# Jamy-L/Handheld-Multi-Frame-Super-Resolution

Measured on AMD Instinct MI355X. Metric: output Mpix/s for 12MP x 20-frame x2 SR burst; max-abs diff vs reference, higher is better.
Workload: dtype f32

## Files before the change

### handheld-multi-frame-super-resolution_amd/csrc/hhsr_kernels.hip

```cpp
#include "hhsr_common.h"


struct CovParams {
    double alpha, beta, k_detail, k_denoise, D_th, D_tr, k_stretch, k_shrink;
    int law;
    double r_D_tr, inv_k_shrink;
};

__device__ __forceinline__ double div_by(double a, double b, double r) {
    const double q = a * r;
    return fma(fma(-b, q, a), r, q);
}

#ifndef HHSR_FAST_SQRT
#define HHSR_FAST_SQRT 1
#endif
__device__ __forceinline__ double sqrt_pos(double t) {
#if HHSR_FAST_SQRT
    const double y = __builtin_amdgcn_rsq(t);
    double g = t * y, h = 0.5 * y;
    const double r = fma(-h, g, 0.5);
    g = fma(g, r, g);
    h = fma(h, r, h);
    const double d = fma(-g, g, t);
    return fma(d, h, g);
#else
    return sqrt(t);
#endif
}

#ifndef HHSR_FAST_DIV
#define HHSR_FAST_DIV 1
#endif
__device__ __forceinline__ float div_f32(float x, float y) {
#if HHSR_FAST_DIV
    const float r = __builtin_amdgcn_rcpf(y), q = x * r;
    return fmaf(fmaf(-y, q, x), r, q);
#else
    return x / y;
#endif
}

__device__ __forceinline__ float gat1(float v, double alpha, double c0, double two_over_alpha) {
    const double t = fmax(alpha * (double)v + c0, 1.0e-300);
    return (float)(two_over_alpha * sqrt_pos(t));
}

template <int SGP>
__device__ __forceinline__ float4 quad_cov(const float* __restrict__ sg, int ly, int lx, int qy, int qx, int gh, int gw,
                                           const CovParams& P) {
    float T00 = 0.f, T01 = 0.f, T11 = 0.f;
#pragma unroll
    for (int i = 0; i < 2; ++i) {
#pragma unroll
        for (int j = 0; j < 2; ++j) {
            const int gy_ = qy - 1 + i, gx_ = qx - 1 + j;
            if (gy_ >= 0 && gy_ < gh - 1 && gx_ >= 0 && gx_ < gw - 1) {
                const float g00 = sg[(ly + i) * SGP + lx + j], g01 = sg[(ly + i) * SGP + lx + j + 1];
                const float g10 = sg[(ly + i + 1) * SGP + lx + j], g11 = sg[(ly + i + 1) * SGP + lx + j + 1];
                const float t0a = -0.5f * g00 + 0.5f * g01, t0b = -0.5f * g10 + 0.5f * g11;
                const float t1a = 0.5f * g00 + 0.5f * g01, t1b = 0.5f * g10 + 0.5f * g11;
                const float vx = 0.5f * t0a + 0.5f * t0b;
                const float vy = -0.5f * t1a + 0.5f * t1b;
                T00 += vx * vx;
                T01 += vx * vy;
                T11 += vy * vy;
            }
        }
    }
    const float b = -(T00 + T11);
    const float c = T00 * T11 - T01 * T01;
    const float bb = b * b;
    double delta = (double)bb - 4.0 * (double)c;
    delta = delta > 0.0 ? delta : 0.0;
    const double sq = delta > 0.0 ? sqrt_pos(delta) : 0.0;
    const double r1 = (-(double)b + sq) / 2.0, r2 = (-(double)b - sq) / 2.0;
    float l1, l2;
    if (fabs(r1) >= fabs(r2)) {
        l1 = (float)r1;
        l2 = (float)r2;
    } else {
        l1 = (float)r2;
        l2 = (float)r1;
    }
    float e1x, e1y, e2x, e2y;
    if (T01 == 0.f && T00 == T11) {
        e1x = 1.f; e1y = 0.f; e2x = 0.f; e2y = 1.f;
    } else {
        const float a0 = T00 + T01 - l2, a1 = T01 + T11 - l2;
        if (a0 == 0.f) {
            e1x = a0; e1y = 1.f; e2x = 1.f; e2y = 0.f;
        } else if (a1 == 0.f) {
            e1x = 1.f; e1y = a1; e2x = 0.f; e2y = 1.f;
        } else {
            const float nrm = sqrtf(a0 * a0 + a1 * a1);
            e1x = div_f32(a0, nrm);
            e1y = div_f32(a1, nrm);
            const float sgn = copysignf(1.f, e1x);
            e2y = fabsf(e1x);
            e2x = -e1y * sgn;
        }
    }
    const double A = 1.0 + (double)sqrtf(div_f32(l1 - l2, l1 + l2));
    double D = 1.0 - div_by((double)sqrtf(l1), P.D_tr, P.r_D_tr) + P.D_th;
    D = D > 0.0 ? D : 0.0;
    D = D < 1.0 ? D : 1.0;
    double k1d, k2d;
    if (P.law == 0) {
        if (A > 1.95) {
            k1d = P.inv_k_shrink;
            k2d = P.k_stretch;
        } else {
            k1d = 1.0;
            k2d = 1.0;
        }
    } else {
        k1d = 1.0 + A / 2.0 * (P.inv_k_shrink - 1.0);
        k2d = 1.0 + A / 2.0 * (P.k_stretch - 1.0);
    }
    const float k1 = (float)(P.k_detail * ((1.0 - D) * k1d + D * P.k_denoise));
    const float k2 = (float)(P.k_detail * ((1.0 - D) * k2d + D * P.k_denoise));
    const float k1s = k1 * k1, k2s = k2 * k2;
    float4 o;
    o.x = k1s * e1x * e1x + k2s * e2x * e2x;
    o.y = k1s * e1x * e1y + k2s * e2x * e2y;
    o.z = o.y;
    o.w = k1s * e1y * e1y + k2s * e2y * e2y;
    return o;
}

constexpr int FS_TX = 32, FS_TY = 16, FS_P = FS_TX + 2 + 1, FS_N = (FS_TY + 2) * (FS_TX + 2);
constexpr int FS_IT = (FS_N + 255) / 256;

struct FsCfa {
    uint8_t c[4];
};
struct FsFrames {
    const float* raw[HHSR_MAX_BATCH];
    float* means[HHSR_MAX_BATCH];
    float* vars[HHSR_MAX_BATCH];
    float4* covs[HHSR_MAX_BATCH];
};

struct FrameStatsArgs {
    const float* raw;
    int pitch, gh, gw;
    FsCfa cfa;
    double rwb[3];
    double rwbk[4];
    int pat;
    int unit_wb;
    float* means;
    float* vars;
    float4* covs;
    CovParams P;
};

template <bool STATS, bool COV>
__global__ void __launch_bounds__(256) k_frame_stats(FrameStatsArgs A, FsFrames fr) {
    A.raw = fr.raw[blockIdx.z];
    A.means = fr.means[blockIdx.z];
    A.vars = fr.vars[blockIdx.z];
    A.covs = fr.covs[blockIdx.z];
    __shared__ float s_ch[STATS ? 3 : 1][STATS ? FS_TY + 2 : 1][FS_P];
    __shared__ float s_g[COV ? (FS_TY + 2) * FS_P : 1];
    const int bid = xcd_remap(blockIdx.y * gridDim.x + blockIdx.x, gridDim.x * gridDim.y);
    const int qx0 = (bid % gridDim.x) * FS_TX, qy0 = (bid / gridDim.x) * FS_TY;
    const int gh = A.gh, gw = A.gw;
    const double c0 = 3.0 / 8.0 * A.P.alpha * A.P.alpha + A.P.beta;
    const double toa = 2.0 / A.P.alpha;
    float2 va[FS_IT], vb[FS_IT];
#pragma unroll
    for (int u = 0; u < FS_IT; ++u) {
        const int p = min(threadIdx.x + 256 * u, FS_N - 1);
        const int i = p / (FS_TX + 2), j = p - i * (FS_TX + 2);
        const int qy = clampi(qy0 + i - 1, 0, gh - 1), qx = clampi(qx0 + j - 1, 0, gw - 1);
        va[u] = *reinterpret_cast<const float2*>(A.raw + (size_t)(2 * qy) * A.pitch + 2 * qx);
        vb[u] = *reinterpret_cast<const float2*>(A.raw + (size_t)(2 * qy + 1) * A.pitch + 2 * qx);
    }
#pragma unroll
    for (int u = 0; u < FS_IT; ++u) {
        const int p = threadIdx.x + 256 * u;
        if (p < FS_N) {
            const int i = p / (FS_TX + 2), j = p - i * (FS_TX + 2);
            const float v[4] = {va[u].x, va[u].y, vb[u].x, vb[u].y};
            if (STATS) {
                float ch[3] = {0.f, 0.f, 0.f};
                const double x0 = (double)v[0] * A.rwbk[0], x1 = (double)v[1] * A.rwbk[1];
                const double x2 = (double)v[2] * A.rwbk[2], x3 = (double)v[3] * A.rwbk[3];
                if (A.unit_wb && A.pat >= 0) {
                    const float g01 = 0.5f * (v[1] + v[2]), g03 = 0.5f * (v[0] + v[3]);
                    ch[1] = A.pat <= 1 ? g01 : g03;
                    ch[0] = A.pat == 0 ? v[0] : A.pat == 1 ? v[3] : A.pat == 2 ? v[1] : v[2];
                    ch[2] = A.pat == 0 ? v[3] : A.pat == 1 ? v[0] : A.pat == 2 ? v[2] : v[1];
                } else if (A.pat == 0) {
                    ch[0] = (float)x0; ch[1] = (float)(((0.0 + x1) + x2) / 2.0); ch[2] = (float)x3;
                } else if (A.pat == 1) {
                    ch[2] = (float)x0; ch[1] = (float)(((0.0 + x1) + x2) / 2.0); ch[0] = (float)x3;
                } else if (A.pat == 2) {
                    ch[0] = (float)x1; ch[1] = (float)(((0.0 + x0) + x3) / 2.0); ch[2] = (float)x2;
                } else if (A.pat == 3) {
                    ch[2] = (float)x1; ch[1] = (float)(((0.0 + x0) + x3) / 2.0); ch[0] = (float)x2;
                } else {
                    double g = 0.0;
                    const double x[4] = {x0, x1, x2, x3};
#pragma unroll
                    for (int k = 0; k < 4; ++k) {
                        const int c = A.cfa.c[k];
                        if (c == 1) g += x[k];
                        else ch[c] = (float)x[k];
                    }
                    ch[1] = (float)(g / 2.0);
                }
                s_ch[0][i][j] = ch[0];
                s_ch[1][i][j] = ch[1];
                s_ch[2][i][j] = ch[2];
            }
            if (COV) {
                const int qy = qy0 + i - 1, qx = qx0 + j - 1;
                float g = 0.f;
                if (qy >= 0 && qy < gh && qx >= 0 && qx < gw) {
                    const double s = (double)gat1(v[0], A.P.alpha, c0, toa) + (double)gat1(v[1], A.P.alpha, c0, toa) +
                                     (double)gat1(v[2], A.P.alpha, c0, toa) + (double)gat1(v[3], A.P.alpha, c0, toa);
                    g = (float)(s / 4.0);
                }
                s_g[i * FS_P + j] = g;
            }
        }
    }
    __syncthreads();
    const int lx = threadIdx.x % FS_TX, ly0 = threadIdx.x / FS_TX;
    const int gx = qx0 + lx;
    if (gx >= gw) return;
    const size_t plane = (size_t)gh * gw;
#pragma unroll
    for (int h = 0; h < 2; ++h) {
        const int ly = ly0 + 8 * h, gy = qy0 + ly;
        if (gy >= gh) break;
        const size_t o = (size_t)gy * gw + gx;
        if (STATS) {
#pragma unroll
            for (int c = 0; c < 3; ++c) {
                float s0 = 0.f, s1 = 0.f;
#pragma unroll
                for (int i = 0; i < 3; ++i)
#pragma unroll
                    for (int j = 0; j < 3; ++j) {
                        const float v = s_ch[c][ly + i][lx + j];
                        s0 += v;
                        s1 += v * v;
                    }
                const float r9 = 1.0f / 9.0f, q9 = s0 * r9;
                A.means[c * plane + o] = fmaf(fmaf(-9.0f, q9, s0), r9, q9);
                if (A.vars) {
                    const double m = div_by((double)s0, 9.0, 1.0 / 9.0);
                    A.vars[c * plane + o] = (float)(div_by((double)s1, 9.0, 1.0 / 9.0) - m * m);
                }
            }
        }
        if (COV) A.covs[o] = quad_cov<FS_P>(s_g, ly, lx, gy, gx, gh, gw, A.P);
    }
}

static int frame_stats_launch_batch(const float* const* raws, int n_frames, int H, int W, int pitch, const uint8_t* cfa,
                                    const double* wb, float* const* means, float* const* vars, float* const* covs,
                                    const CovParams& P, void* stream) {
    FrameStatsArgs A;
    A.raw = nullptr; A.pitch = pitch; A.gh = H / 2; A.gw = W / 2;
    for (int k = 0; k < 4; ++k) A.cfa.c[k] = cfa ? cfa[k] : 0;
    for (int k = 0; k < 3; ++k) A.rwb[k] = wb ? 1.0 / wb[k] : 1.0;
    for (int k = 0; k < 4; ++k) A.rwbk[k] = A.rwb[A.cfa.c[k]];
    const int code = A.cfa.c[0] * 27 + A.cfa.c[1] * 9 + A.cfa.c[2] * 3 + A.cfa.c[3];
    A.pat = code == 0 * 27 + 1 * 9 + 1 * 3 + 2 ? 0 : code == 2 * 27 + 1 * 9 + 1 * 3 + 0 ? 1
          : code == 1 * 27 + 0 * 9 + 2 * 3 + 1 ? 2 : code == 1 * 27 + 2 * 9 + 0 * 3 + 1 ? 3 : -1;
    A.unit_wb = A.rwb[0] == 1.0 && A.rwb[1] == 1.0 && A.rwb[2] == 1.0;
    A.means = nullptr; A.vars = nullptr; A.covs = nullptr; A.P = P;
    A.P.r_D_tr = 1.0 / P.D_tr;
    A.P.inv_k_shrink = 1.0 / P.k_shrink;
    hipStream_t s = (hipStream_t)stream;
    for (int n0 = 0; n0 < n_frames; n0 += HHSR_MAX_BATCH) {
        const int nb = n_frames - n0 < HHSR_MAX_BATCH ? n_frames - n0 : HHSR_MAX_BATCH;
        FsFrames fr;
        for (int k = 0; k < HHSR_MAX_BATCH; ++k) {
            const int n = n0 + (k < nb ? k : 0);
            fr.raw[k] = raws[n];
            fr.means[k] = means ? means[n] : nullptr;
            fr.vars[k] = vars ? vars[n] : nullptr;
            fr.covs[k] = covs ? reinterpret_cast<float4*>(covs[n]) : nullptr;
        }
        const dim3 grid(hhsr_cdiv(A.gw, FS_TX), hhsr_cdiv(A.gh, FS_TY), nb), block(256);
        if (means && covs) hipLaunchKernelGGL((k_frame_stats<true, true>), grid, block, 0, s, A, fr);
        else if (means) hipLaunchKernelGGL((k_frame_stats<true, false>), grid, block, 0, s, A, fr);
        else hipLaunchKernelGGL((k_frame_stats<false, true>), grid, block, 0, s, A, fr);
    }
    return hhsr_launch_status("hhsr_frame_stats");
}

static int frame_stats_launch(const float* raw, int H, int W, int pitch, const uint8_t* cfa, const double* wb,
                              float* means, float* vars, float* covs, const CovParams& P, void* stream) {
    return frame_stats_launch_batch(&raw, 1, H, W, pitch, cfa, wb, means ? &means : nullptr, vars ? &vars : nullptr,
                                    covs ? &covs : nullptr, P, stream);
}

extern "C" int hhsr_cov_from_raw(const float* raw, int H, int W, int pitch, float* covs, double alpha, double beta,
                                 double k_detail, double k_denoise, double D_th, double D_tr, double k_stretch,
                                 double k_shrink, int law, void* stream) {
    HHSR_ARG(raw && covs && H >= 2 && W >= 2 && pitch >= W);
    HHSR_ARG((pitch & 1) == 0 && ((uintptr_t)raw & 7) == 0 && ((uintptr_t)covs & 15) == 0);
    HHSR_ARG(alpha > 0.0);
    HHSR_ARG(law == 0 || law == 1);
    CovParams P{alpha, beta, k_detail, k_denoise, D_th, D_tr, k_stretch, k_shrink, law};
    return frame_stats_launch(raw, H, W, pitch, nullptr, nullptr, nullptr, nullptr, covs, P, stream);
}

extern "C" int hhsr_rob_stats(const float* raw, int H, int W, int pitch, const uint8_t cfa[4], const double* wb,
                              float* means, float* vars, void* stream) {
    HHSR_ARG(raw && cfa && wb && means && H >= 2 && W >= 2 && pitch >= W);
    HHSR_ARG((pitch & 1) == 0 && ((uintptr_t)raw & 7) == 0);
    for (int k = 0; k < 4; ++k) HHSR_ARG(cfa[k] <= 2);
    for (int k = 0; k < 3; ++k) HHSR_ARG(wb[k] != 0.0);
    CovParams P{1.0, 0.0, 0, 0, 0, 1.0, 0, 1.0, 0};
    return frame_stats_launch(raw, H, W, pitch, cfa, wb, means, vars, nullptr, P, stream);
}

extern "C" int hhsr_frame_stats(const float* raw, int H, int W, int pitch, const uint8_t cfa[4], const double* wb,
                                float* means, float* vars, float* covs, double alpha, double beta, double k_detail,
                                double k_denoise, double D_th, double D_tr, double k_stretch, double k_shrink, int law,
                                void* stream) {
    HHSR_ARG(raw && cfa && wb && means && covs && H >= 2 && W >= 2 && pitch >= W);
    HHSR_ARG((pitch & 1) == 0 && ((uintptr_t)raw & 7) == 0 && ((uintptr_t)covs & 15) == 0);
    HHSR_ARG(alpha > 0.0 && (law == 0 || law == 1));
    for (int k = 0; k < 4; ++k) HHSR_ARG(cfa[k] <= 2);
    for (int k = 0; k < 3; ++k) HHSR_ARG(wb[k] != 0.0);
    CovParams P{alpha, beta, k_detail, k_denoise, D_th, D_tr, k_stretch, k_shrink, law};
    return frame_stats_launch(raw, H, W, pitch, cfa, wb, means, vars, covs, P, stream);
}

extern "C" int hhsr_frame_stats_batch(const float* const* raws, int n_frames, int H, int W, int pitch, const uint8_t cfa[4],
                                      const double* wb, float* const* means, float* const* covs, double alpha,
                                      double beta, double k_detail, double k_denoise, double D_th, double D_tr,
                                      double k_stretch, double k_shrink, int law, void* stream) {
    HHSR_ARG(raws && cfa && wb && means && covs && n_frames >= 0 && H >= 2 && W >= 2 && pitch >= W && (pitch & 1) == 0);
    for (int n = 0; n < n_frames; ++n)
        HHSR_ARG(raws[n] && means[n] && covs[n] && ((uintptr_t)raws[n] & 7) == 0 && ((uintptr_t)covs[n] & 15) == 0);
    HHSR_ARG(alpha > 0.0 && (law == 0 || law == 1));
    for (int k = 0; k < 4; ++k) HHSR_ARG(cfa[k] <= 2);
    for (int k = 0; k < 3; ++k) HHSR_ARG(wb[k] != 0.0);
    CovParams P{alpha, beta, k_detail, k_denoise, D_th, D_tr, k_stretch, k_shrink, law};
    return frame_stats_launch_batch(raws, n_frames, H, W, pitch, cfa, wb, means, nullptr, covs, P, stream);
}

struct MonoStatsArgs {
    const float* raw;
    int pitch, H, W;
    float* means;
    float* vars;
    float4* covs;
    CovParams P;
};

template <bool STATS, bool COV>
__global__ void __launch_bounds__(256) k_mono_stats(MonoStatsArgs A) {
    __shared__ float s_v[STATS ? FS_TY + 2 : 1][FS_P];
    __shared__ float s_g[COV ? (FS_TY + 2) * FS_P : 1];
    const int bid = xcd_remap(blockIdx.y * gridDim.x + blockIdx.x, gridDim.x * gridDim.y);
    const int x0 = (bid % gridDim.x) * FS_TX, y0 = (bid / gridDim.x) * FS_TY;
    const int H = A.H, W = A.W;
    const double c0 = 3.0 / 8.0 * A.P.alpha * A.P.alpha + A.P.beta;
    const double toa = 2.0 / A.P.alpha;
    float v[FS_IT];
#pragma unroll
    for (int u = 0; u < FS_IT; ++u) {
        const int p = min(threadIdx.x + 256 * u, FS_N - 1);
        const int i = p / (FS_TX + 2), j = p - i * (FS_TX + 2);
        v[u] = A.raw[(size_t)clampi(y0 + i - 1, 0, H - 1) * A.pitch + clampi(x0 + j - 1, 0, W - 1)];
    }
#pragma unroll
    for (int u = 0; u < FS_IT; ++u) {
        const int p = threadIdx.x + 256 * u;
        if (p < FS_N) {
            const int i = p / (FS_TX + 2), j = p - i * (FS_TX + 2);
            if (STATS) s_v[i][j] = v[u];
            if (COV) {
                const int y = y0 + i - 1, x = x0 + j - 1;
                s_g[i * FS_P + j] = (y >= 0 && y < H && x >= 0 && x < W) ? gat1(v[u], A.P.alpha, c0, toa) : 0.f;
            }
        }
    }
    __syncthreads();
    const int lx = threadIdx.x % FS_TX, ly0 = threadIdx.x / FS_TX;
    const int gx = x0 + lx;
    if (gx >= W) return;
#pragma unroll
    for (int h = 0; h < 2; ++h) {
        const int ly = ly0 + 8 * h, gy = y0 + ly;
        if (gy >= H) break;
        const size_t o = (size_t)gy * W + gx;
        if (STATS) {
            float s0 = 0.f, s1 = 0.f;
#pragma unroll
            for (int i = 0; i < 3; ++i)
#pragma unroll
                for (int j = 0; j < 3; ++j) {
                    const float t = s_v[ly + i][lx + j];
                    s0 += t;
                    s1 += t * t;
                }
            const float r9 = 1.0f / 9.0f, q9 = s0 * r9;
            A.means[o] = fmaf(fmaf(-9.0f, q9, s0), r9, q9);
            if (A.vars) {
                const double m = div_by((double)s0, 9.0, 1.0 / 9.0);
                A.vars[o] = (float)(div_by((double)s1, 9.0, 1.0 / 9.0) - m * m);
            }
        }
        if (COV) A.covs[o] = quad_cov<FS_P>(s_g, ly, lx, gy, gx, H, W, A.P);
    }
}

extern "C" int hhsr_mono_frame_stats(const float* raw, int H, int W, int pitch, float* means, float* vars, float* covs,
                                     double alpha, double beta, double k_detail, double k_denoise, double D_th,
                                     double D_tr, double k_stretch, double k_shrink, int law, void* stream) {
    HHSR_ARG(raw && (means || covs) && H >= 2 && W >= 2 && pitch >= W);
    HHSR_ARG(!vars || means);
    HHSR_ARG(!covs || (((uintptr_t)covs & 15) == 0 && alpha > 0.0 && (law == 0 || law == 1)));
    MonoStatsArgs A;
    A.raw = raw; A.pitch = pitch; A.H = H; A.W = W;
    A.means = means; A.vars = vars; A.covs = reinterpret_cast<float4*>(covs);
    A.P = covs ? CovParams{alpha, beta, k_detail, k_denoise, D_th, D_tr, k_stretch, k_shrink, law}
               : CovParams{1.0, 0.0, 0, 0, 0, 1.0, 0, 1.0, 0};
    A.P.r_D_tr = 1.0 / A.P.D_tr;
    A.P.inv_k_shrink = 1.0 / A.P.k_shrink;
    const dim3 grid(hhsr_cdiv(W, FS_TX), hhsr_cdiv(H, FS_TY)), block(256);
    hipStream_t s = (hipStream_t)stream;
    if (means && covs) hipLaunchKernelGGL((k_mono_stats<true, true>), grid, block, 0, s, A);
    else if (means) hipLaunchKernelGGL((k_mono_stats<true, false>), grid, block, 0, s, A);
    else hipLaunchKernelGGL((k_mono_stats<false, true>), grid, block, 0, s, A);
    return hhsr_launch_status("hhsr_mono_frame_stats");
}
```

Before: 6148.

## Share per-sample gradient outer products in shared memory and enlarge frame-stats tile

The frame-stats kernel now computes each 2x2 gradient outer product once per tile into shared memory, so neighbouring output pixels reuse it instead of each pixel recomputing four samples. The tile height grows from 16 to 24 rows to cut halo overhead, and the mono kernel keeps its old tile constants. The cost is an extra shared buffer, a second barrier and larger register and LDS use per block, which may lower occupancy.

```diff
diff --git a/handheld-multi-frame-super-resolution_amd/csrc/hhsr_kernels.hip b/handheld-multi-frame-super-resolution_amd/csrc/hhsr_kernels.hip
--- a/handheld-multi-frame-super-resolution_amd/csrc/hhsr_kernels.hip
+++ b/handheld-multi-frame-super-resolution_amd/csrc/hhsr_kernels.hip
@@ -46,28 +46,21 @@
     return (float)(two_over_alpha * sqrt_pos(t));
 }
 
+struct CovSample {
+    float xx, xy, yy;
+};
 template <int SGP>
-__device__ __forceinline__ float4 quad_cov(const float* __restrict__ sg, int ly, int lx, int qy, int qx, int gh, int gw,
-                                           const CovParams& P) {
-    float T00 = 0.f, T01 = 0.f, T11 = 0.f;
-#pragma unroll
-    for (int i = 0; i < 2; ++i) {
-#pragma unroll
-        for (int j = 0; j < 2; ++j) {
-            const int gy_ = qy - 1 + i, gx_ = qx - 1 + j;
-            if (gy_ >= 0 && gy_ < gh - 1 && gx_ >= 0 && gx_ < gw - 1) {
-                const float g00 = sg[(ly + i) * SGP + lx + j], g01 = sg[(ly + i) * SGP + lx + j + 1];
-                const float g10 = sg[(ly + i + 1) * SGP + lx + j], g11 = sg[(ly + i + 1) * SGP + lx + j + 1];
-                const float t0a = -0.5f * g00 + 0.5f * g01, t0b = -0.5f * g10 + 0.5f * g11;
-                const float t1a = 0.5f * g00 + 0.5f * g01, t1b = 0.5f * g10 + 0.5f * g11;
-                const float vx = 0.5f * t0a + 0.5f * t0b;
-                const float vy = -0.5f * t1a + 0.5f * t1b;
-                T00 += vx * vx;
-                T01 += vx * vy;
-                T11 += vy * vy;
-            }
-        }
-    }
+__device__ __forceinline__ CovSample cov_sample(const float* __restrict__ sg, int sy, int sx) {
+    const float g00 = sg[sy * SGP + sx], g01 = sg[sy * SGP + sx + 1];
+    const float g10 = sg[(sy + 1) * SGP + sx], g11 = sg[(sy + 1) * SGP + sx + 1];
+    const float t0a = -0.5f * g00 + 0.5f * g01, t0b = -0.5f * g10 + 0.5f * g11;
+    const float t1a = 0.5f * g00 + 0.5f * g01, t1b = 0.5f * g10 + 0.5f * g11;
+    const float vx = 0.5f * t0a + 0.5f * t0b;
+    const float vy = -0.5f * t1a + 0.5f * t1b;
+    return {vx * vx, vx * vy, vy * vy};
+}
+
+__device__ __forceinline__ float4 cov_from_tensor(float T00, float T01, float T11, const CovParams& P) {
     const float b = -(T00 + T11);
     const float c = T00 * T11 - T01 * T01;
     const float bb = b * b;
@@ -129,8 +122,32 @@
     return o;
 }
 
-constexpr int FS_TX = 32, FS_TY = 16, FS_P = FS_TX + 2 + 1, FS_N = (FS_TY + 2) * (FS_TX + 2);
+template <int SGP>
+__device__ __forceinline__ float4 quad_cov(const float* __restrict__ sg, int ly, int lx, int qy, int qx, int gh, int gw,
+                                           const CovParams& P) {
+    float T00 = 0.f, T01 = 0.f, T11 = 0.f;
+#pragma unroll
+    for (int i = 0; i < 2; ++i) {
+#pragma unroll
+        for (int j = 0; j < 2; ++j) {
+            const int gy_ = qy - 1 + i, gx_ = qx - 1 + j;
+            if (gy_ >= 0 && gy_ < gh - 1 && gx_ >= 0 && gx_ < gw - 1) {
+                const CovSample t = cov_sample<SGP>(sg, ly + i, lx + j);
+                T00 += t.xx;
+                T01 += t.xy;
+                T11 += t.yy;
+            }
+        }
+    }
+    return cov_from_tensor(T00, T01, T11, P);
+}
+
+constexpr int FS_TX = 32, FS_TY = 24, FS_P = FS_TX + 2 + 1, FS_N = (FS_TY + 2) * (FS_TX + 2);
 constexpr int FS_IT = (FS_N + 255) / 256;
+constexpr int FS_Q = FS_TY / 8;
+constexpr int FS_SP = FS_TX + 1, FS_SN = (FS_TY + 1) * FS_SP;
+constexpr int FS_SX = FS_TX + FS_TY + 1;
+static_assert(FS_TY % 8 == 0 && FS_SX <= 128, "k_frame_stats: 8 rows of 32 threads; threads 128 .. form the extra samples");
 
 struct FsCfa {
     uint8_t c[4];
@@ -164,6 +181,7 @@
     A.covs = fr.covs[blockIdx.z];
     __shared__ float s_ch[STATS ? 3 : 1][STATS ? FS_TY + 2 : 1][FS_P];
     __shared__ float s_g[COV ? (FS_TY + 2) * FS_P : 1];
+    __shared__ float s_t[3][COV ? FS_SN : 1];
     const int bid = xcd_remap(blockIdx.y * gridDim.x + blockIdx.x, gridDim.x * gridDim.y);
     const int qx0 = (bid % gridDim.x) * FS_TX, qy0 = (bid / gridDim.x) * FS_TY;
     const int gh = A.gh, gw = A.gw;
@@ -230,11 +248,26 @@
     }
     __syncthreads();
     const int lx = threadIdx.x % FS_TX, ly0 = threadIdx.x / FS_TX;
+    if (COV) {
+        auto put = [&](int sy, int sx) {
+            const int gsy = qy0 - 1 + sy, gsx = qx0 - 1 + sx;
+            CovSample t = {0.f, 0.f, 0.f};
+            if (gsy >= 0 && gsy < gh - 1 && gsx >= 0 && gsx < gw - 1) t = cov_sample<FS_P>(s_g, sy, sx);
+            s_t[0][sy * FS_SP + sx] = t.xx;
+            s_t[1][sy * FS_SP + sx] = t.xy;
+            s_t[2][sy * FS_SP + sx] = t.yy;
+        };
+#pragma unroll
+        for (int h = 0; h < FS_Q; ++h) put(ly0 + 8 * h, lx);
+        const int e = (int)threadIdx.x - 128;
+        if (e >= 0 && e < FS_SX) put(e <= FS_TX ? FS_TY : e - (FS_TX + 1), e <= FS_TX ? e : FS_TX);
+        __syncthreads();
+    }
     const int gx = qx0 + lx;
     if (gx >= gw) return;
     const size_t plane = (size_t)gh * gw;
 #pragma unroll
-    for (int h = 0; h < 2; ++h) {
+    for (int h = 0; h < FS_Q; ++h) {
         const int ly = ly0 + 8 * h, gy = qy0 + ly;
         if (gy >= gh) break;
         const size_t o = (size_t)gy * gw + gx;
@@ -258,7 +291,19 @@
                 }
             }
         }
-        if (COV) A.covs[o] = quad_cov<FS_P>(s_g, ly, lx, gy, gx, gh, gw, A.P);
+        if (COV) {
+            float T00 = 0.f, T01 = 0.f, T11 = 0.f;
+#pragma unroll
+            for (int i = 0; i < 2; ++i)
+#pragma unroll
+                for (int j = 0; j < 2; ++j) {
+                    const int k = (ly + i) * FS_SP + lx + j;
+                    T00 += s_t[0][k];
+                    T01 += s_t[1][k];
+                    T11 += s_t[2][k];
+                }
+            A.covs[o] = cov_from_tensor(T00, T01, T11, A.P);
+        }
     }
 }
 
@@ -350,6 +395,9 @@
     return frame_stats_launch_batch(raws, n_frames, H, W, pitch, cfa, wb, means, nullptr, covs, P, stream);
 }
 
+constexpr int MS_TX = 32, MS_TY = 16, MS_P = MS_TX + 2 + 1, MS_N = (MS_TY + 2) * (MS_TX + 2);
+constexpr int MS_IT = (MS_N + 255) / 256;
+
 struct MonoStatsArgs {
     const float* raw;
     int pitch, H, W;
@@ -361,34 +409,34 @@
 
 template <bool STATS, bool COV>
 __global__ void __launch_bounds__(256) k_mono_stats(MonoStatsArgs A) {
-    __shared__ float s_v[STATS ? FS_TY + 2 : 1][FS_P];
-    __shared__ float s_g[COV ? (FS_TY + 2) * FS_P : 1];
+    __shared__ float s_v[STATS ? MS_TY + 2 : 1][MS_P];
+    __shared__ float s_g[COV ? (MS_TY + 2) * MS_P : 1];
     const int bid = xcd_remap(blockIdx.y * gridDim.x + blockIdx.x, gridDim.x * gridDim.y);
-    const int x0 = (bid % gridDim.x) * FS_TX, y0 = (bid / gridDim.x) * FS_TY;
+    const int x0 = (bid % gridDim.x) * MS_TX, y0 = (bid / gridDim.x) * MS_TY;
     const int H = A.H, W = A.W;
     const double c0 = 3.0 / 8.0 * A.P.alpha * A.P.alpha + A.P.beta;
     const double toa = 2.0 / A.P.alpha;
-    float v[FS_IT];
-#pragma unroll
-    for (int u = 0; u < FS_IT; ++u) {
-        const int p = min(threadIdx.x + 256 * u, FS_N - 1);
-        const int i = p / (FS_TX + 2), j = p - i * (FS_TX + 2);
+    float v[MS_IT];
+#pragma unroll
+    for (int u = 0; u < MS_IT; ++u) {
+        const int p = min(threadIdx.x + 256 * u, MS_N - 1);
+        const int i = p / (MS_TX + 2), j = p - i * (MS_TX + 2);
         v[u] = A.raw[(size_t)clampi(y0 + i - 1, 0, H - 1) * A.pitch + clampi(x0 + j - 1, 0, W - 1)];
     }
 #pragma unroll
-    for (int u = 0; u < FS_IT; ++u) {
+    for (int u = 0; u < MS_IT; ++u) {
         const int p = threadIdx.x + 256 * u;
-        if (p < FS_N) {
-            const int i = p / (FS_TX + 2), j = p - i * (FS_TX + 2);
+        if (p < MS_N) {
+            const int i = p / (MS_TX + 2), j = p - i * (MS_TX + 2);
             if (STATS) s_v[i][j] = v[u];
             if (COV) {
                 const int y = y0 + i - 1, x = x0 + j - 1;
-                s_g[i * FS_P + j] = (y >= 0 && y < H && x >= 0 && x < W) ? gat1(v[u], A.P.alpha, c0, toa) : 0.f;
+                s_g[i * MS_P + j] = (y >= 0 && y < H && x >= 0 && x < W) ? gat1(v[u], A.P.alpha, c0, toa) : 0.f;
             }
         }
     }
     __syncthreads();
-    const int lx = threadIdx.x % FS_TX, ly0 = threadIdx.x / FS_TX;
+    const int lx = threadIdx.x % MS_TX, ly0 = threadIdx.x / MS_TX;
     const int gx = x0 + lx;
     if (gx >= W) return;
 #pragma unroll
@@ -413,7 +461,7 @@
                 A.vars[o] = (float)(div_by((double)s1, 9.0, 1.0 / 9.0) - m * m);
             }
         }
-        if (COV) A.covs[o] = quad_cov<FS_P>(s_g, ly, lx, gy, gx, H, W, A.P);
+        if (COV) A.covs[o] = quad_cov<MS_P>(s_g, ly, lx, gy, gx, H, W, A.P);
     }
 }
 
@@ -430,7 +478,7 @@
                : CovParams{1.0, 0.0, 0, 0, 0, 1.0, 0, 1.0, 0};
     A.P.r_D_tr = 1.0 / A.P.D_tr;
     A.P.inv_k_shrink = 1.0 / A.P.k_shrink;
-    const dim3 grid(hhsr_cdiv(W, FS_TX), hhsr_cdiv(H, FS_TY)), block(256);
+    const dim3 grid(hhsr_cdiv(W, MS_TX), hhsr_cdiv(H, MS_TY)), block(256);
     hipStream_t s = (hipStream_t)stream;
     if (means && covs) hipLaunchKernelGGL((k_mono_stats<true, true>), grid, block, 0, s, A);
     else if (means) hipLaunchKernelGGL((k_mono_stats<true, false>), grid, block, 0, s, A);
```

Result: faster. 6216 (median of 6 runs) (+1.1%).
